# huangzh13/StyleGAN.pytorch

Hardware: AMD Instinct MI355X
Metric: img/s full G+D train step, 1024x1024 depth-9 bf16 (higher is better)
Workload: dtype bf16; 1 GPU; ffhq1024: StyleGAN 1024x1024, progressive depth index 8, logistic+R1, alpha 0.5, batch 4/GPU, global batch 4; global_batch=4, parallelism=dp1

## Files before the change

stylegan/pytorch_amd/csrc/pointwise.hip:

```cpp
#include "common.h"

static inline unsigned grid_for(size_t nvec, int block = 256) {
    size_t g = (nvec + block - 1) / block;
    static const size_t cap = [] { const char* e = getenv("SGX_GRID_CAP"); const long v = e ? atol(e) : 8192; return (size_t)(v > 0 ? v : 0x7fffffffL); }();
    if (g > cap) g = cap;
    if (g < 1) g = 1;
    return (unsigned)g;
}
static inline unsigned grid_all(size_t nvec, int block = 256) {
    size_t g = (nvec + block - 1) / block;
    static const size_t cap = [] { const char* e = getenv("SGX_GRID_ALL_CAP"); const long v = e ? atol(e) : 0; return (size_t)(v > 0 ? v : 0x7fffffffL); }();
    if (g > cap) g = cap;
    if (g < 1) g = 1;
    return (unsigned)g;
}

template <typename T>
__global__ void bias_act_kernel(const T* __restrict__ x, const float* __restrict__ bias, float bscale, T* __restrict__ y,
                                size_t nvec, int C, int act) {
    constexpr int VE = VecTraits<T>::VE;
    const int cv = C / VE;
    for (size_t i = (size_t)blockIdx.x * blockDim.x + threadIdx.x; i < nvec; i += (size_t)gridDim.x * blockDim.x) {
        float v[VE];
        VecTraits<T>::load(x + i * VE, v);
        const int c0 = (int)(i % cv) * VE;
#pragma unroll
        for (int j = 0; j < VE; ++j) {
            float t = v[j] + (bias ? bscale * bias[c0 + j] : 0.f);
            v[j] = act_apply(t, act);
        }
        VecTraits<T>::store(y + i * VE, v);
    }
}
__global__ void bias_act_scalar_kernel(const float* __restrict__ x, const float* __restrict__ bias, float bscale, float* __restrict__ y,
                                       size_t n, int C, int act) {
    for (size_t i = (size_t)blockIdx.x * blockDim.x + threadIdx.x; i < n; i += (size_t)gridDim.x * blockDim.x) {
        const float t = x[i] + (bias ? bscale * bias[i % C] : 0.f);
        y[i] = act_apply(t, act);
    }
}
extern "C" int sgx_bias_act(const void* x, const float* bias, float bscale, void* y, size_t npix, int C, int act, int dtype, void* stream) {
    hipStream_t st = (hipStream_t)stream;
    SGX_REQUIRE(act >= SGX_ACT_NONE && act <= SGX_ACT_RELU, SGX_EINVAL, "bias_act: activation %d", act);
    SGX_NOTE(0.0, 2.0 * (dtype == SGX_F32 ? 4.0 : 2.0) * npix * C, "bias_act %zux%d", npix, C);
    if (dtype == SGX_F32 && C % 4 != 0) {
        hipLaunchKernelGGL(bias_act_scalar_kernel, dim3(grid_for(npix * C)), dim3(256), 0, st, (const float*)x, bias, bscale, (float*)y, npix * C, C, act);
        SGX_LAUNCH_CHECK("bias_act_scalar");
        return 0;
    }
    if (dtype == SGX_F32) {
        SGX_REQUIRE(C % 4 == 0, SGX_EUNSUPPORTED, "bias_act: C %% 4");
        size_t nvec = npix * C / 4;
        hipLaunchKernelGGL(bias_act_kernel<float>, dim3(grid_all(nvec)), dim3(256), 0, st, (const float*)x, bias, bscale, (float*)y, nvec, C, act);
    } else {
// ... 11 lines not shown
    if (scale_dev) scale = scale_dev[0];
    constexpr int VE = VecTraits<T>::VE;
    for (size_t i = (size_t)blockIdx.x * blockDim.x + threadIdx.x; i < nvec; i += (size_t)gridDim.x * blockDim.x) {
        float g[VE], a[VE];
        VecTraits<T>::load(dy + i * VE, g);
        VecTraits<T>::load(y + i * VE, a);
#pragma unroll
        for (int j = 0; j < VE; ++j) g[j] = (scale * g[j]) * (a[j] > 0.f ? 1.f : slope);
        VecTraits<T>::store(dx + i * VE, g);
    }
}
extern "C" int sgx_lrelu_bwd(const void* dy, const void* y, void* dx, size_t n, float slope, float scale, const float* scale_dev, int dtype,
                             void* stream) {
    hipStream_t st = (hipStream_t)stream;
    SGX_NOTE(0.0, 3.0 * (dtype == SGX_F32 ? 4.0 : 2.0) * n, "lrelu_bwd %zu", n);
    if (dtype == SGX_F32) {
        SGX_REQUIRE(n % 4 == 0, SGX_EUNSUPPORTED, "lrelu_bwd: n %% 4");
        hipLaunchKernelGGL(lrelu_bwd_kernel<float>, dim3(grid_all(n / 4)), dim3(256), 0, st, (const float*)dy, (const float*)y, (float*)dx, n / 4, slope, scale, scale_dev);
    } else {
        SGX_REQUIRE(n % 8 == 0, SGX_EUNSUPPORTED, "lrelu_bwd: n %% 8");
        hipLaunchKernelGGL(lrelu_bwd_kernel<bf16_t>, dim3(grid_all(n / 8)), dim3(256), 0, st, (const bf16_t*)dy, (const bf16_t*)y, (bf16_t*)dx, n / 8, slope, scale, scale_dev);
    }
    SGX_LAUNCH_CHECK("lrelu_bwd");
    return 0;
}

__global__ void lrelu_bwd_bits_kernel(const bf16_t* __restrict__ dy, const unsigned char* __restrict__ bits, bf16_t* __restrict__ dx, size_t nvec, float slope,
                                      float scale, const float* __restrict__ scale_dev, int nt) {
    if (scale_dev) scale = scale_dev[0];
    for (size_t i = (size_t)blockIdx.x * blockDim.x + threadIdx.x; i < nvec; i += (size_t)gridDim.x * blockDim.x) {
        float g[8];
        const uint4 raw = ld16(dy + i * 8, nt != 0);
        const unsigned w4[4] = {raw.x, raw.y, raw.z, raw.w};
#pragma unroll
        for (int k = 0; k < 4; ++k) { g[2 * k] = __uint_as_float(w4[k] << 16); g[2 * k + 1] = __uint_as_float(w4[k] & 0xffff0000u); }
        const unsigned bb = bits[i];
#pragma unroll
        for (int j = 0; j < 8; ++j) g[j] = (scale * g[j]) * (((bb >> j) & 1u) ? 1.f : slope);
        st16(dx + i * 8, make_uint4(pack_bf16x2(g[0], g[1]), pack_bf16x2(g[2], g[3]), pack_bf16x2(g[4], g[5]), pack_bf16x2(g[6], g[7])), nt != 0);
    }
}
extern "C" int sgx_lrelu_bwd_bits(const void* dy, const void* bits, void* dx, size_t n, float slope, float scale, const float* scale_dev, int dtype,
                                  void* stream) {
    SGX_REQUIRE(dtype == SGX_BF16 && n % 8 == 0, SGX_EUNSUPPORTED, "lrelu_bwd_bits: bf16, n %% 8 == 0");
    SGX_REQUIRE(dy && bits && dx, SGX_EINVAL, "lrelu_bwd_bits: null argument");
    SGX_NOTE(0.0, 4.125 * n, "lrelu_bwd_bits %zu", n);
    hipLaunchKernelGGL(lrelu_bwd_bits_kernel, dim3(grid_all(n / 8)), dim3(256), 0, (hipStream_t)stream, (const bf16_t*)dy, (const unsigned char*)bits, (bf16_t*)dx,
                       n / 8, slope, scale, scale_dev, sgx_nt_for(2.0 * (double)n) ? 1 : 0);
    SGX_LAUNCH_CHECK("lrelu_bwd_bits");
    return 0;
}

#define FRB_BLOCKS 2048
template <int CV>
__global__ __launch_bounds__(256) void fade_rgb_bwd_kernel(const bf16_t* __restrict__ g, const unsigned char* __restrict__ bits, const float* __restrict__ pimg,
                                                           const float* __restrict__ wr, float ws, float alpha, float beta, const float* __restrict__ ab_dev,
                                                           bf16_t* __restrict__ gy, float* __restrict__ gpimg, double* __restrict__ part, size_t npix, int nt) {
    constexpr int PPI = 256 / CV;
    __shared__ double sh[4][CV][32];
    if (ab_dev) { alpha = ab_dev[0]; beta = ab_dev[1]; }
    const int tid = threadIdx.x, v = tid % CV, pl = tid / CV, lane = tid & 63, wave = tid >> 6;
    const size_t per = (npix + gridDim.x - 1) / gridDim.x;
    const size_t p0 = (size_t)blockIdx.x * per, p1 = p0 + per < npix ? p0 + per : npix;
    float wv[8][3];
    if (gpimg) {
#pragma unroll
        for (int j = 0; j < 8; ++j)
#pragma unroll
            for (int k = 0; k < 3; ++k) wv[j][k] = (beta * ws) * wr[(v * 8 + j) * 3 + k];
    }
    double acc[8][4];
    float q[8][4];
#pragma unroll
    for (int j = 0; j < 8; ++j)
#pragma unroll
        for (int k = 0; k < 4; ++k) { acc[j][k] = 0.0; q[j][k] = 0.f; }
    int cnt = 0;
    for (size_t pb = p0; pb < p1; pb += PPI) {
        const size_t p = pb + pl;
        const bool ok = p < p1;
        float gv[8];
        float i0 = 0.f, i1 = 0.f, i2 = 0.f;
        unsigned bb = 0;
        if (ok) {
            {
                const uint4 raw = ld16(g + (p * CV + v) * 8, nt != 0);
                const unsigned w4[4] = {raw.x, raw.y, raw.z, raw.w};
#pragma unroll
                for (int i = 0; i < 4; ++i) { gv[2 * i] = __uint_as_float(w4[i] << 16); gv[2 * i + 1] = __uint_as_float(w4[i] & 0xffff0000u); }
            }
            bb = bits[p * CV + v];
            i0 = pimg[p * 3]; i1 = pimg[p * 3 + 1]; i2 = pimg[p * 3 + 2];
            float o[8];
#pragma unroll
            for (int j = 0; j < 8; ++j) o[j] = (alpha * gv[j]) * (((bb >> j) & 1u) ? 1.f : SGX_LRELU);
            st16(gy + (p * CV + v) * 8, make_uint4(pack_bf16x2(o[0], o[1]), pack_bf16x2(o[2], o[3]), pack_bf16x2(o[4], o[5]), pack_bf16x2(o[6], o[7])), nt != 0);
        } else {
#pragma unroll
            for (int j = 0; j < 8; ++j) gv[j] = 0.f;
        }
#pragma unroll
        for (int j = 0; j < 8; ++j) { q[j][0] += gv[j] * i0; q[j][1] += gv[j] * i1; q[j][2] += gv[j] * i2; q[j][3] += gv[j]; }
        if (++cnt == 64) {
#pragma unroll
            for (int j = 0; j < 8; ++j)
#pragma unroll
                for (int k = 0; k < 4; ++k) { acc[j][k] += (double)q[j][k]; q[j][k] = 0.f; }
            cnt = 0;
        }
        if (gpimg) {
            float s0 = 0.f, s1 = 0.f, s2 = 0.f;
#pragma unroll
            for (int j = 0; j < 8; ++j) { s0 += gv[j] * wv[j][0]; s1 += gv[j] * wv[j][1]; s2 += gv[j] * wv[j][2]; }
#pragma unroll
            for (int o = 1; o < CV; o <<= 1) { s0 += __shfl_xor(s0, o, 64); s1 += __shfl_xor(s1, o, 64); s2 += __shfl_xor(s2, o, 64); }
            if (ok && v == 0) { gpimg[p * 3] = s0; gpimg[p * 3 + 1] = s1; gpimg[p * 3 + 2] = s2; }
        }
    }
#pragma unroll
    for (int j = 0; j < 8; ++j)
#pragma unroll
        for (int k = 0; k < 4; ++k) {
            double t = acc[j][k] + (double)q[j][k];
#pragma unroll
            for (int o = CV; o < 64; o <<= 1) t += __shfl_xor(t, o, 64);
            if (lane < CV) sh[wave][lane][j * 4 + k] = t;
        }
    __syncthreads();
    for (int e = tid; e < CV * 32; e += 256) {
        const int vv = e / 32, r = e % 32;
        part[((size_t)blockIdx.x * CV + vv) * 32 + r] = (sh[0][vv][r] + sh[1][vv][r]) + (sh[2][vv][r] + sh[3][vv][r]);
    }
}
__global__ __launch_bounds__(256) void fade_rgb_bwd_finish(const double* __restrict__ part, float* __restrict__ dw, float* __restrict__ drb, int nblk, int C,
                                                           float ws, float bs, float beta, const float* __restrict__ ab_dev, int acc) {
    __shared__ double sh[64][5];
    if (ab_dev) beta = ab_dev[1];
    const int el = threadIdx.x & 3, pl = threadIdx.x >> 2;
    const int e = blockIdx.x * 4 + el;
    double s = 0.0;
    if (e < 4 * C)
        for (int b = pl; b < nblk; b += 64) s += part[(size_t)b * 4 * C + e];
    sh[pl][el] = s;
    __syncthreads();
    if (pl == 0 && e < 4 * C) {
        double t = 0.0;
        for (int k = 0; k < 64; ++k) t += sh[k][el];
        const int c = e >> 2, j = e & 3;
        if (j < 3) {
            if (dw) { const float val = (float)(t * ((double)beta * (double)ws)); dw[c * 3 + j] = (acc & 1) ? dw[c * 3 + j] + val : val; }
        } else if (drb) {
            const float val = (float)(t * ((double)beta * (double)bs));
            drb[c] = (acc & 2) ? drb[c] + val : val;
        }
    }
}
extern "C" size_t sgx_fade_rgb_bwd_ws_bytes(size_t npix, int C) { (void)npix; return (size_t)FRB_BLOCKS * 4 * C * sizeof(double); }
extern "C" int sgx_fade_rgb_bwd(const void* g, const void* bits, const float* pimg, const float* wr, float ws, float bs, float alpha, float beta,
                                const float* ab_dev, void* gy, float* dwr, float* drb, int acc, float* gpimg, void* wsbuf, size_t ws_bytes, size_t npix, int C,
                                int dtype, void* stream) {
    SGX_REQUIRE(dtype == SGX_BF16 && (C == 32 || C == 64 || C == 128), SGX_EUNSUPPORTED, "fade_rgb_bwd: bf16, C in {32, 64, 128} (C=%d dtype %d)", C, dtype);
    SGX_REQUIRE(g && bits && pimg && wr && gy && wsbuf && npix > 0, SGX_EINVAL, "fade_rgb_bwd: null argument");
    SGX_REQUIRE(ws_bytes >= sgx_fade_rgb_bwd_ws_bytes(npix, C), SGX_EWORKSPACE, "fade_rgb_bwd: workspace");
    SGX_NOTE(8.0 * npix * C, npix * (4.125 * C + 12.0 + (gpimg ? 12.0 : 0.0)), "fade_rgb_bwd %zux%d", npix, C);
    hipStream_t st = (hipStream_t)stream;
    const int ppi = 256 / (C / 8);
    long nblk = (long)((npix + (size_t)ppi * 8 - 1) / ((size_t)ppi * 8));
    if (nblk > FRB_BLOCKS) nblk = FRB_BLOCKS;
    if (nblk < 1) nblk = 1;
    const bf16_t* gp = static_cast<const bf16_t*>(g);
    const unsigned char* bp = static_cast<const unsigned char*>(bits);
    bf16_t* yp = static_cast<bf16_t*>(gy);
    double* part = static_cast<double*>(wsbuf);
    const int nt = sgx_nt_for(2.0 * (double)npix * C) ? 1 : 0;
    if (C == 32) hipLaunchKernelGGL(fade_rgb_bwd_kernel<4>, dim3((unsigned)nblk), dim3(256), 0, st, gp, bp, pimg, wr, ws, alpha, beta, ab_dev, yp, gpimg, part, npix, nt);
    else if (C == 64) hipLaunchKernelGGL(fade_rgb_bwd_kernel<8>, dim3((unsigned)nblk), dim3(256), 0, st, gp, bp, pimg, wr, ws, alpha, beta, ab_dev, yp, gpimg, part, npix, nt);
    else hipLaunchKernelGGL(fade_rgb_bwd_kernel<16>, dim3((unsigned)nblk), dim3(256), 0, st, gp, bp, pimg, wr, ws, alpha, beta, ab_dev, yp, gpimg, part, npix, nt);
    SGX_LAUNCH_CHECK("fade_rgb_bwd_kernel");
    if (dwr || drb) {
        hipLaunchKernelGGL(fade_rgb_bwd_finish, dim3((unsigned)((4 * C + 3) / 4)), dim3(256), 0, st, part, dwr, drb, (int)nblk, C, ws, bs, beta, ab_dev, acc);
        SGX_LAUNCH_CHECK("fade_rgb_bwd_finish");
    }
    return 0;
}
extern "C" int sgx_fade_rgb_bwd_finish(const void* wsbuf, size_t ws_bytes, size_t npix, int C, float ws, float bs, float beta, const float* ab_dev,
                                       float* dwr, float* drb, int acc, void* stream) {
    SGX_REQUIRE(C == 32 || C == 64 || C == 128, SGX_EUNSUPPORTED, "fade_rgb_bwd_finish: C in {32, 64, 128} (C=%d)", C);
    SGX_REQUIRE(wsbuf && npix > 0 && (dwr || drb), SGX_EINVAL, "fade_rgb_bwd_finish: null argument");
    SGX_REQUIRE(ws_bytes >= sgx_fade_rgb_bwd_ws_bytes(npix, C), SGX_EWORKSPACE, "fade_rgb_bwd_finish: workspace");
    const int ppi = 256 / (C / 8);
    long nblk = (long)((npix + (size_t)ppi * 8 - 1) / ((size_t)ppi * 8));
    if (nblk > FRB_BLOCKS) nblk = FRB_BLOCKS;
    if (nblk < 1) nblk = 1;
    SGX_NOTE(0.0, (double)nblk * 4 * C * sizeof(double), "fade_rgb_bwd_finish C%d", C);
    hipLaunchKernelGGL(fade_rgb_bwd_finish, dim3((unsigned)((4 * C + 3) / 4)), dim3(256), 0, (hipStream_t)stream, static_cast<const double*>(wsbuf), dwr, drb,
                       (int)nblk, C, ws, bs, beta, ab_dev, acc);
    SGX_LAUNCH_CHECK("fade_rgb_bwd_finish");
    return 0;
}

__global__ __launch_bounds__(256) void fade_rgb_bwd2_kernel(const bf16_t* __restrict__ ggy, const float* __restrict__ ggp, const unsigned char* __restrict__ bits,
                                                            const float* __restrict__ wr, float ws, float alpha, float beta, const float* __restrict__ ab_dev,
                                                            bf16_t* __restrict__ out, size_t npix, int C) {
    const int cv = C / 8;
    const size_t nvec = npix * cv;
    const size_t i0 = (size_t)blockIdx.x * blockDim.x + threadIdx.x;
    const int c0 = (int)(i0 % cv) * 8;
    if (ab_dev) { alpha = ab_dev[0]; beta = ab_dev[1]; }
    float w0[8], w1[8], w2[8];
#pragma unroll
    for (int j = 0; j < 8; ++j) { w0[j] = ws * wr[(c0 + j) * 3]; w1[j] = ws * wr[(c0 + j) * 3 + 1]; w2[j] = ws * wr[(c0 + j) * 3 + 2]; }
    for (size_t i = i0; i < nvec; i += (size_t)gridDim.x * blockDim.x) {
        const size_t p = i / cv;
        float t1[8], t2[8], o[8];
#pragma unroll
        for (int j = 0; j < 8; ++j) { t1[j] = 0.f; t2[j] = 0.f; }
        if (ggy) {
            float g[8];
            VecTraits<bf16_t>::load(ggy + i * 8, g);
            const unsigned bb = bits[i];
#pragma unroll
            for (int j = 0; j < 8; ++j) t1[j] = bf2f(f2bf((alpha * g[j]) * (((bb >> j) & 1u) ? 1.f : SGX_LRELU)));
        }
        if (ggp) {
            const float r = ggp[p * 3], g = ggp[p * 3 + 1], b = ggp[p * 3 + 2];
#pragma unroll
            for (int j = 0; j < 8; ++j) {
                t2[j] = bf2f(f2bf(0.f + (r * w0[j] + g * w1[j] + b * w2[j])));
                if (ab_dev) t2[j] = bf2f(f2bf(beta * t2[j]));
            }
        }
#pragma unroll
        for (int j = 0; j < 8; ++j) o[j] = t1[j] + t2[j];
        VecTraits<bf16_t>::store(out + i * 8, o);
    }
}
extern "C" int sgx_fade_rgb_bwd2(const void* ggy, const float* ggp, const void* bits, const float* wr, float ws, float alpha, float beta, const float* ab_dev,
                                 void* out, size_t npix, int C, int dtype, void* stream) {
    SGX_REQUIRE(dtype == SGX_BF16 && (C == 32 || C == 64 || C == 128), SGX_EUNSUPPORTED, "fade_rgb_bwd2: bf16, C in {32, 64, 128} (C=%d dtype %d)", C, dtype);
    SGX_REQUIRE((ggy || ggp) && wr && out && npix > 0 && (!ggy || bits), SGX_EINVAL, "fade_rgb_bwd2: null argument");
    SGX_REQUIRE(ab_dev || beta == 1.0f, SGX_EUNSUPPORTED, "fade_rgb_bwd2: a host beta other than 1 rides in ws (as the forward's)");
    SGX_NOTE(6.0 * npix * C, npix * ((ggy ? 4.125 : 2.0) * C + (ggp ? 12.0 : 0.0)), "fade_rgb_bwd2 %zux%d", npix, C);
    const int cv = C / 8;
    unsigned grid = grid_for(npix * cv);
    hipLaunchKernelGGL(fade_rgb_bwd2_kernel, dim3(grid), dim3(256), 0, (hipStream_t)stream, static_cast<const bf16_t*>(ggy), ggp,
                       static_cast<const unsigned char*>(bits), wr, ws, alpha, beta, ab_dev, static_cast<bf16_t*>(out), npix, C);
    SGX_LAUNCH_CHECK("fade_rgb_bwd2_kernel");
    return 0;
}

template <typename T>
__global__ void axpby_kernel(const T* __restrict__ a, const T* __restrict__ b, T* __restrict__ out, float alpha, float beta,
                             const float* __restrict__ alpha_dev, const float* __restrict__ beta_dev, size_t nvec, size_t n) {
    constexpr int VE = VecTraits<T>::VE;
    if (alpha_dev) alpha = alpha_dev[0];
    if (beta_dev) beta = beta_dev[0];
    for (size_t i = (size_t)blockIdx.x * blockDim.x + threadIdx.x; i < nvec; i += (size_t)gridDim.x * blockDim.x) {
        if ((i + 1) * VE <= n) {
            float va[VE], vb[VE];
            VecTraits<T>::load(a + i * VE, va);
            if (b) {
                VecTraits<T>::load(b + i * VE, vb);
#pragma unroll
                for (int j = 0; j < VE; ++j) va[j] = alpha * va[j] + beta * vb[j];
            } else {
#pragma unroll
                for (int j = 0; j < VE; ++j) va[j] = alpha * va[j];
            }
            VecTraits<T>::store(out + i * VE, va);
        } else {
            for (size_t k = i * VE; k < n; ++k) {
                float t = alpha * to_f(a[k]) + (b ? beta * to_f(b[k]) : 0.f);
                out[k] = from_f<T>(t);
            }
        }
    }
}
static int axpby_launch(const void* a, const void* b, void* out, float alpha, float beta, const float* alpha_dev, const float* beta_dev,
                        size_t n, int dtype, void* stream) {
    hipStream_t st = (hipStream_t)stream;
    SGX_NOTE(0.0, (b ? 3.0 : 2.0) * (dtype == SGX_F32 ? 4.0 : 2.0) * n, "axpby %zu", n);
    if (n == 0) return 0;
    if (dtype == SGX_F32) {
        size_t nvec = (n + 3) / 4;
        hipLaunchKernelGGL(axpby_kernel<float>, dim3(grid_all(nvec)), dim3(256), 0, st, (const float*)a, (const float*)b, (float*)out, alpha, beta, alpha_dev, beta_dev, nvec, n);
    } else {
        size_t nvec = (n + 7) / 8;
        hipLaunchKernelGGL(axpby_kernel<bf16_t>, dim3(grid_all(nvec)), dim3(256), 0, st, (const bf16_t*)a, (const bf16_t*)b, (bf16_t*)out, alpha, beta, alpha_dev, beta_dev, nvec, n);
// ... 1041 lines not shown
    if (dtype == SGX_F32) hipLaunchKernelGGL(rgb_out_kernel<float>, dim3(g), dim3(256), sh, st, (const float*)x, w, sj, sc, wscale, bias, img, npix, C, lpp, low, H, W, alpha, beta, ab_dev);
    else hipLaunchKernelGGL(rgb_out_kernel<bf16_t>, dim3(g), dim3(256), sh, st, (const bf16_t*)x, w, sj, sc, wscale, bias, img, npix, C, lpp, low, H, W, alpha, beta, ab_dev);
    SGX_LAUNCH_CHECK("rgb_out");
    return 0;
}
extern "C" int sgx_rgb_out(const void* x, const float* w, int sj, int sc, float wscale, const float* bias, float* img, size_t npix, int C, int dtype, void* stream) {
    SGX_NOTE(6.0 * npix * C, npix * (12.0 + (dtype == SGX_F32 ? 4.0 : 2.0) * C), "rgb_out %zux%d", npix, C);
    return rgb_out_launch(x, w, sj, sc, wscale, bias, img, npix, C, dtype, nullptr, 1, 1, 1.f, 0.f, nullptr, (hipStream_t)stream);
}
extern "C" int sgx_rgb_out_fade(const void* x, const float* w, int sj, int sc, float wscale, const float* bias, const float* low, float alpha,
                                float beta, const float* ab_dev, float* img, int B, int H, int W, int C, int dtype, void* stream) {
    SGX_REQUIRE(x && w && low && img && B > 0 && H > 0 && W > 0 && H % 2 == 0 && W % 2 == 0, SGX_EINVAL, "rgb_out_fade: bad arguments (%dx%d)", H, W);
    const size_t npix = (size_t)B * H * W;
    SGX_NOTE(6.0 * npix * C, npix * (12.0 + 3.0 + (dtype == SGX_F32 ? 4.0 : 2.0) * C), "rgb_out+fade %zux%d", npix, C);
    return rgb_out_launch(x, w, sj, sc, wscale, bias, img, npix, C, dtype, low, H, W, alpha, beta, ab_dev, (hipStream_t)stream);
}

template <typename T>
__global__ __launch_bounds__(256) void rgb_out_epi_kernel(const T* __restrict__ y, const float* __restrict__ ebias, const float* __restrict__ noise,
                                                          const float* __restrict__ nw, const float* __restrict__ style, const float* __restrict__ mean,
                                                          const float* __restrict__ rstd, const float* __restrict__ w, int sj, int sc, float wscale,
                                                          const float* __restrict__ rbias, float* __restrict__ img, int HW, int C, int lpp,
                                                          const float* __restrict__ low, int Himg, int Wimg, float alpha, float beta,
                                                          const float* __restrict__ ab_dev) {
    constexpr int VE = VecTraits<T>::VE;
    extern __shared__ float sw[];
    if (ab_dev) { alpha = ab_dev[0]; beta = ab_dev[1]; }
    float* kb = sw + 3 * C; float* kw = kb + C; float* sb = kw + C; float* red = sb + 4;
    const int b = blockIdx.y;
    float c0 = 0.f, c1 = 0.f, c2 = 0.f;
    for (int c = threadIdx.x; c < C; c += blockDim.x) {
        const float s0 = style ? style[(size_t)b * 2 * C + c] : 0.f, s1 = style ? style[(size_t)b * 2 * C + C + c] : 0.f;
        const float A = rstd[(size_t)b * C + c] * (s0 + 1.f), S = s1 - mean[(size_t)b * C + c] * A;
        const float w0 = (alpha * wscale) * w[c * sc], w1 = (alpha * wscale) * w[sj + c * sc], w2 = (alpha * wscale) * w[2 * sj + c * sc];
        sw[c] = w0 * A; sw[C + c] = w1 * A; sw[2 * C + c] = w2 * A;
        c0 += w0 * S; c1 += w1 * S; c2 += w2 * S;
        kb[c] = ebias ? ebias[c] : 0.f; kw[c] = nw[c];
    }
    red[threadIdx.x * 3] = c0; red[threadIdx.x * 3 + 1] = c1; red[threadIdx.x * 3 + 2] = c2;
    __syncthreads();
    if (threadIdx.x < 3) {
        float t = 0.f;
        for (int k = 0; k < 256; ++k) t += red[k * 3 + threadIdx.x];
        sb[threadIdx.x] = t + (rbias ? alpha * rbias[threadIdx.x] : 0.f);
    }
    __syncthreads();
    const float b0 = sb[0], b1 = sb[1], b2 = sb[2];
    const int cv = C / VE;
    const int sub = threadIdx.x % lpp;
    const int gid = (blockIdx.x * blockDim.x + threadIdx.x) / lpp, gstride = (gridDim.x * blockDim.x) / lpp;
    const T* yb = y + (size_t)b * HW * C;
    const float* nzb = noise + (size_t)b * HW;
    const int niter = (HW + gstride - 1) / gstride;
    for (int it = 0; it < niter; ++it) {
        const int p = gid + it * gstride;
        float s0 = 0.f, s1 = 0.f, s2 = 0.f;
        if (p < HW) {
            const float nz = nzb[p];
            for (int v = sub; v < cv; v += lpp) {
                float t[VE];
                VecTraits<T>::load(yb + ((size_t)p * cv + v) * VE, t);
#pragma unroll
                for (int q = 0; q < VE; ++q) {
                    const int c = v * VE + q;
                    const float a = lrelu(t[q] + kb[c] + kw[c] * nz);
                    s0 += a * sw[c]; s1 += a * sw[C + c]; s2 += a * sw[2 * C + c];
                }
            }
        }
        for (int o = lpp >> 1; o > 0; o >>= 1) {
            s0 += __shfl_xor(s0, o, 64); s1 += __shfl_xor(s1, o, 64); s2 += __shfl_xor(s2, o, 64);
        }
        if (p < HW && sub == 0) {
            float o0 = s0 + b0, o1 = s1 + b1, o2 = s2 + b2;
            if (low) {
                const int xw = p % Wimg, yy = p / Wimg;
                const float* l = low + (((size_t)b * (Himg >> 1) + (yy >> 1)) * (Wimg >> 1) + (xw >> 1)) * 3;
                o0 += beta * l[0]; o1 += beta * l[1]; o2 += beta * l[2];
            }
            float* o = img + ((size_t)b * HW + p) * 3;
            o[0] = o0; o[1] = o1; o[2] = o2;
        }
    }
}
extern "C" int sgx_rgb_out_epi(const void* y, const float* ebias, const float* noise, const float* nw, const float* style, const float* mean,
                               const float* rstd, const float* w, int sj, int sc, float wscale, const float* rbias, const float* low, float alpha,
                               float beta, const float* ab_dev, float* img, int B, int H, int W, int C, int dtype, void* stream) {
    SGX_REQUIRE(y && noise && nw && mean && rstd && w && img && B > 0 && H > 0 && W > 0, SGX_EINVAL, "rgb_out_epi: bad arguments");
    SGX_REQUIRE(!low || (H % 2 == 0 && W % 2 == 0), SGX_EINVAL, "rgb_out_epi: odd size %dx%d with a low-resolution image", H, W);
    const int ve = dtype == SGX_F32 ? 4 : 8;
    SGX_REQUIRE((dtype == SGX_F32 || dtype == SGX_BF16) && C % ve == 0 && C <= 2048, SGX_EUNSUPPORTED, "rgb_out_epi: C=%d", C);
    int lpp = C / ve;
    if (lpp > 16) lpp = 16;
    SGX_REQUIRE((lpp & (lpp - 1)) == 0, SGX_EUNSUPPORTED, "rgb_out_epi: C=%d", C);
    const int HW = H * W;
    const double npix = (double)B * HW;
    SGX_NOTE(8.0 * npix * C, npix * (12.0 + 4.0 + (low ? 3.0 : 0.0) + (dtype == SGX_F32 ? 4.0 : 2.0) * C), "epi+rgb_out%s %.0fx%d", low ? "+fade" : "", npix, C);
    long bx = ((long)HW * lpp + 255) / 256;
    const long cap = 4096 / B > 1 ? 4096 / B : 1;
    if (bx > cap) bx = cap;
    const size_t sh = (size_t)(5 * C + 4 + 256 * 3) * sizeof(float);
    hipStream_t st = (hipStream_t)stream;
    if (dtype == SGX_F32)
        hipLaunchKernelGGL(rgb_out_epi_kernel<float>, dim3((unsigned)bx, (unsigned)B), dim3(256), sh, st, (const float*)y, ebias, noise, nw, style, mean, rstd, w, sj, sc,
                           wscale, rbias, img, HW, C, lpp, low, H, W, alpha, beta, ab_dev);
    else
// ... 179 lines not shown
```

stylegan/pytorch_amd/csrc/rgbconv.hip:

```cpp
#include "common.h"
#include <stdlib.h>

typedef __attribute__((ext_vector_type(4))) float f32x4_t;

typedef _Float16 h16x4 __attribute__((ext_vector_type(4)));
typedef _Float16 h16x2 __attribute__((ext_vector_type(2)));
typedef float f32x2 __attribute__((ext_vector_type(2)));
static __device__ __forceinline__ unsigned pack_f16x2(float lo, float hi) {
    const h16x2 v = {(_Float16)lo, (_Float16)hi};
    return __builtin_bit_cast(unsigned, v);
}
static __device__ __forceinline__ f32x4_t mma16h(s16x4 a, s16x4 b, f32x4_t c) {
    return __builtin_amdgcn_mfma_f32_16x16x16f16(__builtin_bit_cast(h16x4, a), __builtin_bit_cast(h16x4, b), c, 0, 0, 0);
}
static __device__ __forceinline__ f32x4_t mma16(s16x4 a, s16x4 b, f32x4_t c) {
    return __builtin_amdgcn_mfma_f32_16x16x16bf16_1k(a, b, c, 0, 0, 0);
}

__global__ void rgbconv_pack_kernel(const float* __restrict__ w0, float s0, const float* __restrict__ wr, float sr,
                                    const float* __restrict__ br, float bscale, bf16_t* __restrict__ wf, bf16_t* __restrict__ wd, int C) {
    const int tid = threadIdx.x + blockIdx.x * blockDim.x, nth = blockDim.x * gridDim.x;
    for (int e = tid; e < 3 * C * 16; e += nth) {
        const int ky = e / (C * 16), o = (e / 16) % C, k = e % 16, kx = k >> 2, j = k & 3;
        float v = 0.f;
// ... 294 lines not shown
                    a[2 * q] = fmaxf(p.x, n.x); a[2 * q + 1] = fmaxf(p.y, n.y);
                }
                unsigned nib = 0u;
#pragma unroll
                for (int i = 0; i < 4; ++i)
                    nib |= (unsigned)min(max(__float_as_int(a[i]), 0), 1) << i;
                const auto sw = __builtin_amdgcn_permlane16_swap(nib, nib, false, false);
                float h[4];
#pragma unroll
                for (int i = 0; i < 4; ++i) {
                    const float t = a[i] + dpp_row_shr1(a[i]);
                    h[i] = t + dpp_row_shl1(t);
                }
                const f32x2 vc0 = f32x2{h1[cb][0], h1[cb][1]} + f32x2{h[0], h[1]}, vc1 = f32x2{h1[cb][2], h1[cb][3]} + f32x2{h[2], h[3]};
                if (store_row) {
                    if (y_out) {
                        const f32x2 o0 = vp[cb][0] + vc0, o1 = vp[cb][1] + vc1;
                        *reinterpret_cast<uint2*>(yrow + yoff + cb * 16) = make_uint2(pack_bf16x2(o0.x, o0.y), pack_bf16x2(o1.x, o1.y));
                    }
                    if (bit_out) brow[boff + cb * 2] = (unsigned char)pbyte[cb];
                }
                vp[cb][0] = vc0; vp[cb][1] = vc1;
#pragma unroll
                for (int i = 0; i < 4; ++i) h1[cb][i] = h[i];
                pbyte[cb] = sw[0] | (sw[1] << 4);
            }
        }
    }
}
template <int CB>
__global__ __launch_bounds__(256) void rgbconv_fwdblur_kernel(const float* __restrict__ img, const bf16_t* __restrict__ wf, const float* __restrict__ b0,
                                                              bf16_t* __restrict__ y, unsigned char* __restrict__ bits, int B, int H, int W, int ones,
                                                              int nstrips, int nrb, int nit, int dbg) {
    constexpr int C = 16 * CB;
    int item = __builtin_amdgcn_readfirstlane((int)(rc_xcd_block() * 4 + (threadIdx.x >> 6)));
    const int sx = item % nstrips; item /= nstrips;
    const int rbk = item % nrb, b = item / nrb;
    if (b >= B) return;
    const int rb = 6 * nit - 2;
    const int r_begin = rbk * rb, r_end = r_begin + rb < H ? r_begin + rb : H;
    const float* ibase = img + (size_t)b * H * W * 3;
    bf16_t* ybase = y + (size_t)b * H * W * C;
    unsigned char* bbase = bits ? bits + (size_t)b * H * W * (C / 8) : nullptr;
    const bool inside = sx * RC_STRIP - 2 >= 0 && sx * RC_STRIP + 15 < W && r_begin - 2 >= 0 && r_begin + rb + 1 < H;
    if (inside) fwdblur_walk<CB, false>(ibase, wf, b0, ybase, bbase, H, W, ones, sx, r_begin, r_end, nit, dbg);
    else fwdblur_walk<CB, true>(ibase, wf, b0, ybase, bbase, H, W, ones, sx, r_begin, r_end, nit, dbg);
}

template <int CB>
__global__ __launch_bounds__(256) void rgbconv_dgrad_kernel(const bf16_t* __restrict__ gz, const bf16_t* __restrict__ wd, float* __restrict__ gi,
                                                            int B, int H, int W, int nstrips, int nrb) {
    constexpr int C = 16 * CB;
    const int lane = threadIdx.x & 63, l15 = lane & 15, l4 = lane >> 4;
    int item = (int)rc_xcd_block() * 4 + (threadIdx.x >> 6);
    const int sx = item % nstrips; item /= nstrips;
    const int rbk = item % nrb, b = item / nrb;
    if (b >= B) return;
    const int r_begin = rbk * RC_ROWS, r_end = r_begin + RC_ROWS < H ? r_begin + RC_ROWS : H;
    const int pc = sx * RC_STRIP - 1 + l15;
    const bool pc_ok = (unsigned)pc < (unsigned)W;
    s16x4 wfr[3][CB];
#pragma unroll
    for (int ky = 0; ky < 3; ++ky)
#pragma unroll
        for (int cb = 0; cb < CB; ++cb) wfr[ky][cb] = *reinterpret_cast<const s16x4*>(wd + ((ky * 16 + l15) * C + cb * 16 + 4 * l4));
    const bf16_t* gbase = gz + (size_t)b * H * W * C;
    struct Row { uint2 v[CB]; };
    auto load_row = [&](int gy) -> Row {
        Row r;
#pragma unroll
        for (int cb = 0; cb < CB; ++cb) {
            r.v[cb] = make_uint2(0u, 0u);
            if (pc_ok && (unsigned)gy < (unsigned)H) r.v[cb] = *reinterpret_cast<const uint2*>(gbase + ((size_t)gy * W + pc) * C + cb * 16 + 4 * l4);
        }
        return r;
    };
    auto frag_of = [&](const uint2& u) -> s16x4 {
        s16x4 f;
        f[0] = (short)(u.x & 0xffffu); f[1] = (short)(u.x >> 16); f[2] = (short)(u.y & 0xffffu); f[3] = (short)(u.y >> 16);
        return f;
    };
    Row g0 = load_row(r_begin - 1), g1 = load_row(r_begin);
    Row ring[RC_PF];
#pragma unroll
    for (int u = 0; u < RC_PF; ++u) ring[u] = load_row(r_begin + 1 + u);
    const bool col_out = l4 == 1 && l15 >= 1 && l15 <= RC_STRIP && pc < W;
    for (int rb = r_begin; rb < r_end; rb += RC_PF) {
#pragma unroll
        for (int u = 0; u < RC_PF; ++u) {
            const int r = rb + u;
            if (r < r_end) {
                const Row g2 = ring[u];
                ring[u] = load_row(r + 1 + RC_PF);
                f32x4_t acc = f32x4_t{0.f, 0.f, 0.f, 0.f};
#pragma unroll
                for (int cb = 0; cb < CB; ++cb) {
                    acc = mma16(wfr[0][cb], frag_of(g0.v[cb]), acc);
                    acc = mma16(wfr[1][cb], frag_of(g1.v[cb]), acc);
                    acc = mma16(wfr[2][cb], frag_of(g2.v[cb]), acc);
                }
                float o3[3];
#pragma unroll
                for (int j = 0; j < 3; ++j) o3[j] = __shfl(acc[j], l15 - 1, 64) + acc[j] + __shfl(acc[j], 32 + l15 + 1, 64);
                if (col_out) *reinterpret_cast<rgb3*>(gi + (((size_t)b * H + r) * W + pc) * 3) = rgb3{o3[0], o3[1], o3[2]};
                g0 = g1; g1 = g2;
            }
        }
    }
}

template <int CB> struct RcWg {
    static constexpr int C = 16 * CB, TH = 8, TW = 64, TP = TH * TW, RH = TH + 2;
    static constexpr int TPS = TP + 8, IPS = RH * TW + 8;
    static constexpr int GZT = C * TPS * 2;
    static constexpr int IMT = 12 * IPS * 2;
    static constexpr int RED = 4 * CB * 3 * 256 * 4;
    static constexpr int LDS = (GZT + IMT > RED ? GZT + IMT : RED);
    static constexpr int NOUT = C * 48;
};

template <int CB>
__global__ __launch_bounds__(256) void rgbconv_wgrad_kernel(const float* __restrict__ img, const bf16_t* __restrict__ gz, float* __restrict__ part,
                                                            int B, int H, int W, int ones, int tiles_x, int tiles_y, int ntiles) {
    using G = RcWg<CB>;
    constexpr int C = G::C, TH = G::TH, TW = G::TW, TP = G::TP, TPS = G::TPS, IPS = G::IPS, RH = G::RH, VPP = C / 8;
    extern __shared__ __attribute__((aligned(16))) char smem[];
    bf16_t* gzT = reinterpret_cast<bf16_t*>(smem);
    bf16_t* imgT = reinterpret_cast<bf16_t*>(smem + G::GZT);
    const int tid = threadIdx.x, lane = tid & 63, wave = tid >> 6, l15 = lane & 15, l4 = lane >> 4;
    f32x4_t acc[CB][3];
#pragma unroll
    for (int cb = 0; cb < CB; ++cb)
#pragma unroll
        for (int ky = 0; ky < 3; ++ky) acc[cb][ky] = f32x4_t{0.f, 0.f, 0.f, 0.f};
    const int nkx = (l15 >> 2) < 3 ? (l15 >> 2) : 0, nj = l15 & 3;
    const RcSched sc = rc_sched(ntiles);
    constexpr int NGV = TP * VPP / 256;
    constexpr int NIP = RH * (TW + 2), NII = (NIP + 255) / 256;
    uint4 gv[NGV];
    rgb3 iv[NII];
    unsigned okm = 0;
    auto tile_at = [&](int t, int& b, int& ty0, int& tx0) {
        const int tx = t % tiles_x; t /= tiles_x;
        const int ty = t % tiles_y;
        b = t / tiles_y; ty0 = ty * TH; tx0 = tx * TW;
    };
    auto load_tile = [&](int t) {
        int b, ty0, tx0;
        tile_at(t, b, ty0, tx0);
#pragma unroll
        for (int it = 0; it < NGV; ++it) {
            const int idx = it * 256 + tid, p = idx / VPP, v = idx - p * VPP, r = p / TW, c = p - r * TW;
            const int gy = ty0 + r, gx = tx0 + c;
            gv[it] = (gy < H && gx < W) ? *reinterpret_cast<const uint4*>(gz + (((size_t)b * H + gy) * W + gx) * C + v * 8) : make_uint4(0u, 0u, 0u, 0u);
        }
        okm = 0;
#pragma unroll
        for (int it = 0; it < NII; ++it) {
            const int idx = it * 256 + tid, rr = idx / (TW + 2), cr = idx - rr * (TW + 2);
// ... 268 lines not shown
```

Measured before the change: 283.1 img/s.

## Unroll and batch loads in fade-RGB, to-RGB and rgbconv dgrad kernels

Several RGB-path kernels get restructured for more memory-level parallelism. fade_rgb_bwd and fade_rgb_bwd2 now issue loads for several pixel trips before computing, with compile-time variants for full tiles and for the nt and nullable-input cases. fade_rgb_bwd also moves its weights into shared memory and uses DPP lane swizzles for the small reductions. A to-RGB kernel gains an unrolled fast path when the channel split matches, and rgbconv dgrad clamps its addresses so loads are branch-free, masking the out-of-range values afterwards. These changes add more registers and code, and the unconditional dgrad loop runs extra MMA work on tail rows.

```diff
diff --git a/stylegan/pytorch_amd/csrc/pointwise.hip b/stylegan/pytorch_amd/csrc/pointwise.hip
--- a/stylegan/pytorch_amd/csrc/pointwise.hip
+++ b/stylegan/pytorch_amd/csrc/pointwise.hip
@@ -1,5 +1,12 @@
 #include "common.h"
-
+#include <type_traits>
+
+template <int O>
+__device__ __forceinline__ float lane_xor(float v) {
+    if constexpr (O == 1) return __int_as_float(__builtin_amdgcn_mov_dpp(__float_as_int(v), 0xB1, 0xf, 0xf, true));
+    else if constexpr (O == 2) return __int_as_float(__builtin_amdgcn_mov_dpp(__float_as_int(v), 0x4E, 0xf, 0xf, true));
+    else return __shfl_xor(v, O, 64);
+}
 static inline unsigned grid_for(size_t nvec, int block = 256) {
     size_t g = (nvec + block - 1) / block;
     static const size_t cap = [] { const char* e = getenv("SGX_GRID_CAP"); const long v = e ? atol(e) : 8192; return (size_t)(v > 0 ? v : 0x7fffffffL); }();
@@ -117,84 +124,137 @@
 }
 
 #define FRB_BLOCKS 2048
+#define FRB_U 2
+#define FRB_US 4
 template <int CV>
 __global__ __launch_bounds__(256) void fade_rgb_bwd_kernel(const bf16_t* __restrict__ g, const unsigned char* __restrict__ bits, const float* __restrict__ pimg,
                                                            const float* __restrict__ wr, float ws, float alpha, float beta, const float* __restrict__ ab_dev,
                                                            bf16_t* __restrict__ gy, float* __restrict__ gpimg, double* __restrict__ part, size_t npix, int nt) {
     constexpr int PPI = 256 / CV;
     __shared__ double sh[4][CV][32];
+    __shared__ float wv[CV][24];
     if (ab_dev) { alpha = ab_dev[0]; beta = ab_dev[1]; }
     const int tid = threadIdx.x, v = tid % CV, pl = tid / CV, lane = tid & 63, wave = tid >> 6;
     const size_t per = (npix + gridDim.x - 1) / gridDim.x;
     const size_t p0 = (size_t)blockIdx.x * per, p1 = p0 + per < npix ? p0 + per : npix;
-    float wv[8][3];
     if (gpimg) {
+        for (int e = tid; e < CV * 24; e += 256) wv[e / 24][e % 24] = (beta * ws) * wr[e];
+        __syncthreads();
+    }
+    float q[8][4];
+#pragma unroll
+    for (int j = 0; j < 8; ++j)
+#pragma unroll
+        for (int k = 0; k < 4; ++k) q[j][k] = 0.f;
+    auto trips = [&](auto UC, auto NT, auto FULL, size_t pb, auto&& flush) {
+        constexpr int UU = decltype(UC)::value;
+        constexpr bool nth = decltype(NT)::value;
+        constexpr bool full = decltype(FULL)::value;
+        uint4 raw[UU];
+        unsigned bb[UU];
+        float im[UU][3];
+        const uint4* gb = reinterpret_cast<const uint4*>(g) + pb * CV;
+        const unsigned char* bq = bits + pb * CV;
+        const float* ib = pimg + pb * 3;
+#pragma unroll
+        for (int u = 0; u < UU; ++u) {
+            const unsigned pi = (unsigned)(u * PPI + pl);
+            const bool ok = full || pb + pi < p1;
+            const unsigned pc = ok ? pi : (unsigned)(p1 - 1 - pb);
+            const uint4 r = ld16(gb + (pc * CV + v), nth);
+            bb[u] = bq[pc * CV + v];
+            const float a0 = ib[pc * 3], a1 = ib[pc * 3 + 1], a2 = ib[pc * 3 + 2];
+            raw[u] = make_uint4(ok ? r.x : 0u, ok ? r.y : 0u, ok ? r.z : 0u, ok ? r.w : 0u);
+            im[u][0] = ok ? a0 : 0.f; im[u][1] = ok ? a1 : 0.f; im[u][2] = ok ? a2 : 0.f;
+        }
+#pragma unroll
+        for (int u = 0; u < UU; ++u) {
+            const unsigned pi = (unsigned)(u * PPI + pl);
+            const bool ok = full || pb + pi < p1;
+            float gv[8];
+            const unsigned w4[4] = {raw[u].x, raw[u].y, raw[u].z, raw[u].w};
+#pragma unroll
+            for (int i = 0; i < 4; ++i) { gv[2 * i] = __uint_as_float(w4[i] << 16); gv[2 * i + 1] = __uint_as_float(w4[i] & 0xffff0000u); }
+            const float i0 = im[u][0], i1 = im[u][1], i2 = im[u][2];
+            if (ok) {
+                float o[8];
+#pragma unroll
+                for (int j = 0; j < 8; ++j) o[j] = (alpha * gv[j]) * (((bb[u] >> j) & 1u) ? 1.f : SGX_LRELU);
+                st16(reinterpret_cast<uint4*>(gy) + pb * CV + (pi * CV + v),
+                     make_uint4(pack_bf16x2(o[0], o[1]), pack_bf16x2(o[2], o[3]), pack_bf16x2(o[4], o[5]), pack_bf16x2(o[6], o[7])), nth);
+            }
+#pragma unroll
+            for (int j = 0; j < 8; ++j) { q[j][0] += gv[j] * i0; q[j][1] += gv[j] * i1; q[j][2] += gv[j] * i2; q[j][3] += gv[j]; }
+            flush();
+            if (gpimg) {
+                float s0 = 0.f, s1 = 0.f, s2 = 0.f;
+#pragma unroll
+                for (int j = 0; j < 8; ++j) { s0 += gv[j] * wv[v][j * 3]; s1 += gv[j] * wv[v][j * 3 + 1]; s2 += gv[j] * wv[v][j * 3 + 2]; }
+                if constexpr (CV > 1) { s0 += lane_xor<1>(s0); s1 += lane_xor<1>(s1); s2 += lane_xor<1>(s2); }
+                if constexpr (CV > 2) { s0 += lane_xor<2>(s0); s1 += lane_xor<2>(s1); s2 += lane_xor<2>(s2); }
+                if constexpr (CV > 4) { s0 += lane_xor<4>(s0); s1 += lane_xor<4>(s1); s2 += lane_xor<4>(s2); }
+                if constexpr (CV > 8) { s0 += lane_xor<8>(s0); s1 += lane_xor<8>(s1); s2 += lane_xor<8>(s2); }
+                if (ok && v == 0) { float* o = gpimg + pb * 3 + pi * 3; o[0] = s0; o[1] = s1; o[2] = s2; }
+            }
+        }
+    };
+    const size_t span = p0 < p1 ? p1 - p0 : 0, ntrip = (span + PPI - 1) / PPI, nfull = span / PPI;
+    auto walk = [&](auto UC, auto NT, auto&& flush) {
+        constexpr int UU = decltype(UC)::value;
+        size_t t = 0;
+        for (; t + UU <= nfull; t += UU) trips(UC, NT, std::true_type{}, p0 + t * PPI, flush);
+        if constexpr (UU > 2)
+            for (; t + 2 <= nfull; t += 2) trips(std::integral_constant<int, 2>{}, NT, std::true_type{}, p0 + t * PPI, flush);
+        for (; t < ntrip; ++t) trips(std::integral_constant<int, 1>{}, NT, std::false_type{}, p0 + t * PPI, flush);
+    };
+    auto finish = [&](auto&& total) {
+        double t[8][4];
 #pragma unroll
         for (int j = 0; j < 8; ++j)
 #pragma unroll
-            for (int k = 0; k < 3; ++k) wv[j][k] = (beta * ws) * wr[(v * 8 + j) * 3 + k];
-    }
-    double acc[8][4];
-    float q[8][4];
-#pragma unroll
-    for (int j = 0; j < 8; ++j)
-#pragma unroll
-        for (int k = 0; k < 4; ++k) { acc[j][k] = 0.0; q[j][k] = 0.f; }
-    int cnt = 0;
-    for (size_t pb = p0; pb < p1; pb += PPI) {
-        const size_t p = pb + pl;
-        const bool ok = p < p1;
-        float gv[8];
-        float i0 = 0.f, i1 = 0.f, i2 = 0.f;
-        unsigned bb = 0;
-        if (ok) {
-            {
-                const uint4 raw = ld16(g + (p * CV + v) * 8, nt != 0);
-                const unsigned w4[4] = {raw.x, raw.y, raw.z, raw.w};
-#pragma unroll
-                for (int i = 0; i < 4; ++i) { gv[2 * i] = __uint_as_float(w4[i] << 16); gv[2 * i + 1] = __uint_as_float(w4[i] & 0xffff0000u); }
-            }
-            bb = bits[p * CV + v];
-            i0 = pimg[p * 3]; i1 = pimg[p * 3 + 1]; i2 = pimg[p * 3 + 2];
-            float o[8];
-#pragma unroll
-            for (int j = 0; j < 8; ++j) o[j] = (alpha * gv[j]) * (((bb >> j) & 1u) ? 1.f : SGX_LRELU);
-            st16(gy + (p * CV + v) * 8, make_uint4(pack_bf16x2(o[0], o[1]), pack_bf16x2(o[2], o[3]), pack_bf16x2(o[4], o[5]), pack_bf16x2(o[6], o[7])), nt != 0);
-        } else {
-#pragma unroll
-            for (int j = 0; j < 8; ++j) gv[j] = 0.f;
-        }
-#pragma unroll
-        for (int j = 0; j < 8; ++j) { q[j][0] += gv[j] * i0; q[j][1] += gv[j] * i1; q[j][2] += gv[j] * i2; q[j][3] += gv[j]; }
-        if (++cnt == 64) {
+            for (int k = 0; k < 4; ++k) t[j][k] = total(j, k);
+#pragma unroll
+        for (int o = CV; o < 64; o <<= 1)
 #pragma unroll
             for (int j = 0; j < 8; ++j)
 #pragma unroll
-                for (int k = 0; k < 4; ++k) { acc[j][k] += (double)q[j][k]; q[j][k] = 0.f; }
-            cnt = 0;
-        }
-        if (gpimg) {
-            float s0 = 0.f, s1 = 0.f, s2 = 0.f;
-#pragma unroll
-            for (int j = 0; j < 8; ++j) { s0 += gv[j] * wv[j][0]; s1 += gv[j] * wv[j][1]; s2 += gv[j] * wv[j][2]; }
-#pragma unroll
-            for (int o = 1; o < CV; o <<= 1) { s0 += __shfl_xor(s0, o, 64); s1 += __shfl_xor(s1, o, 64); s2 += __shfl_xor(s2, o, 64); }
-            if (ok && v == 0) { gpimg[p * 3] = s0; gpimg[p * 3 + 1] = s1; gpimg[p * 3 + 2] = s2; }
-        }
-    }
-#pragma unroll
-    for (int j = 0; j < 8; ++j)
-#pragma unroll
-        for (int k = 0; k < 4; ++k) {
-            double t = acc[j][k] + (double)q[j][k];
-#pragma unroll
-            for (int o = CV; o < 64; o <<= 1) t += __shfl_xor(t, o, 64);
-            if (lane < CV) sh[wave][lane][j * 4 + k] = t;
-        }
-    __syncthreads();
-    for (int e = tid; e < CV * 32; e += 256) {
-        const int vv = e / 32, r = e % 32;
-        part[((size_t)blockIdx.x * CV + vv) * 32 + r] = (sh[0][vv][r] + sh[1][vv][r]) + (sh[2][vv][r] + sh[3][vv][r]);
+                for (int k = 0; k < 4; ++k) t[j][k] += __shfl_xor(t[j][k], o, 64);
+        if (lane < CV) {
+#pragma unroll
+            for (int j = 0; j < 8; ++j)
+#pragma unroll
+                for (int k = 0; k < 4; ++k) sh[wave][lane][j * 4 + k] = t[j][k];
+        }
+        __syncthreads();
+        for (int e = tid; e < CV * 32; e += 256) {
+            const int vv = e / 32, r = e % 32;
+            part[((size_t)blockIdx.x * CV + vv) * 32 + r] = (sh[0][vv][r] + sh[1][vv][r]) + (sh[2][vv][r] + sh[3][vv][r]);
+        }
+    };
+    if (ntrip < 64) {
+        auto none = [] {};
+        if (nt) walk(std::integral_constant<int, FRB_US>{}, std::true_type{}, none);
+        else walk(std::integral_constant<int, FRB_US>{}, std::false_type{}, none);
+        finish([&](int j, int k) { return 0.0 + (double)q[j][k]; });
+    } else {
+        double acc[8][4];
+#pragma unroll
+        for (int j = 0; j < 8; ++j)
+#pragma unroll
+            for (int k = 0; k < 4; ++k) acc[j][k] = 0.0;
+        int cnt = 0;
+        auto flush = [&] {
+            if (++cnt == 64) {
+#pragma unroll
+                for (int j = 0; j < 8; ++j)
+#pragma unroll
+                    for (int k = 0; k < 4; ++k) { acc[j][k] += (double)q[j][k]; q[j][k] = 0.f; }
+                cnt = 0;
+            }
+        };
+        if (nt) walk(std::integral_constant<int, FRB_U>{}, std::true_type{}, flush);
+        else walk(std::integral_constant<int, FRB_U>{}, std::false_type{}, flush);
+        finish([&](int j, int k) { return acc[j][k] + (double)q[j][k]; });
     }
 }
 __global__ __launch_bounds__(256) void fade_rgb_bwd_finish(const double* __restrict__ part, float* __restrict__ dw, float* __restrict__ drb, int nblk, int C,
@@ -275,30 +335,54 @@
     float w0[8], w1[8], w2[8];
 #pragma unroll
     for (int j = 0; j < 8; ++j) { w0[j] = ws * wr[(c0 + j) * 3]; w1[j] = ws * wr[(c0 + j) * 3 + 1]; w2[j] = ws * wr[(c0 + j) * 3 + 2]; }
-    for (size_t i = i0; i < nvec; i += (size_t)gridDim.x * blockDim.x) {
-        const size_t p = i / cv;
-        float t1[8], t2[8], o[8];
-#pragma unroll
-        for (int j = 0; j < 8; ++j) { t1[j] = 0.f; t2[j] = 0.f; }
-        if (ggy) {
-            float g[8];
-            VecTraits<bf16_t>::load(ggy + i * 8, g);
-            const unsigned bb = bits[i];
-#pragma unroll
-            for (int j = 0; j < 8; ++j) t1[j] = bf2f(f2bf((alpha * g[j]) * (((bb >> j) & 1u) ? 1.f : SGX_LRELU)));
-        }
-        if (ggp) {
-            const float r = ggp[p * 3], g = ggp[p * 3 + 1], b = ggp[p * 3 + 2];
-#pragma unroll
-            for (int j = 0; j < 8; ++j) {
-                t2[j] = bf2f(f2bf(0.f + (r * w0[j] + g * w1[j] + b * w2[j])));
-                if (ab_dev) t2[j] = bf2f(f2bf(beta * t2[j]));
-            }
-        }
-#pragma unroll
-        for (int j = 0; j < 8; ++j) o[j] = t1[j] + t2[j];
-        VecTraits<bf16_t>::store(out + i * 8, o);
-    }
+    const size_t gs = (size_t)gridDim.x * blockDim.x;
+    const int cvs = __ffs(cv) - 1;
+    auto trips = [&](auto UC, auto HY, auto HP, size_t i) {
+        constexpr int UU = decltype(UC)::value;
+        constexpr bool hy = decltype(HY)::value, hp = decltype(HP)::value;
+        uint4 raw[UU];
+        unsigned bb[UU];
+        float pr[UU], pg[UU], pb[UU];
+#pragma unroll
+        for (int u = 0; u < UU; ++u) {
+            const size_t iu = i + u * gs;
+            if constexpr (hy) { raw[u] = *reinterpret_cast<const uint4*>(ggy + iu * 8); bb[u] = bits[iu]; }
+            if constexpr (hp) { const size_t p = iu >> cvs; pr[u] = ggp[p * 3]; pg[u] = ggp[p * 3 + 1]; pb[u] = ggp[p * 3 + 2]; }
+        }
+#pragma unroll
+        for (int u = 0; u < UU; ++u) {
+            float t1[8], t2[8], o[8];
+#pragma unroll
+            for (int j = 0; j < 8; ++j) { t1[j] = 0.f; t2[j] = 0.f; }
+            if constexpr (hy) {
+                const unsigned w4[4] = {raw[u].x, raw[u].y, raw[u].z, raw[u].w};
+                float g[8];
+#pragma unroll
+                for (int k = 0; k < 4; ++k) { g[2 * k] = __uint_as_float(w4[k] << 16); g[2 * k + 1] = __uint_as_float(w4[k] & 0xffff0000u); }
+#pragma unroll
+                for (int j = 0; j < 8; ++j) t1[j] = bf2f(f2bf((alpha * g[j]) * (((bb[u] >> j) & 1u) ? 1.f : SGX_LRELU)));
+            }
+            if constexpr (hp) {
+                const float r = pr[u], g = pg[u], b = pb[u];
+#pragma unroll
+                for (int j = 0; j < 8; ++j) {
+                    t2[j] = bf2f(f2bf(0.f + (r * w0[j] + g * w1[j] + b * w2[j])));
+                    if (ab_dev) t2[j] = bf2f(f2bf(beta * t2[j]));
+                }
+            }
+#pragma unroll
+            for (int j = 0; j < 8; ++j) o[j] = t1[j] + t2[j];
+            VecTraits<bf16_t>::store(out + (i + u * gs) * 8, o);
+        }
+    };
+    auto walk = [&](auto HY, auto HP) {
+        size_t i = i0;
+        for (; i + gs < nvec; i += 2 * gs) trips(std::integral_constant<int, 2>{}, HY, HP, i);
+        if (i < nvec) trips(std::integral_constant<int, 1>{}, HY, HP, i);
+    };
+    if (ggy && ggp) walk(std::true_type{}, std::true_type{});
+    else if (ggy) walk(std::true_type{}, std::false_type{});
+    else walk(std::false_type{}, std::true_type{});
 }
 extern "C" int sgx_fade_rgb_bwd2(const void* ggy, const float* ggp, const void* bits, const float* wr, float ws, float alpha, float beta, const float* ab_dev,
                                  void* out, size_t npix, int C, int dtype, void* stream) {
@@ -1446,6 +1530,60 @@
     const T* yb = y + (size_t)b * HW * C;
     const float* nzb = noise + (size_t)b * HW;
     const int niter = (HW + gstride - 1) / gstride;
+    if (cv == lpp) {
+        float rb[VE], rw[VE], r0[VE], r1[VE], r2[VE];
+#pragma unroll
+        for (int q = 0; q < VE; ++q) { const int c = sub * VE + q; rb[q] = kb[c]; rw[q] = kw[c]; r0[q] = sw[c]; r1[q] = sw[C + c]; r2[q] = sw[2 * C + c]; }
+        auto trips = [&](auto UC, int it) {
+            constexpr int UU = decltype(UC)::value;
+            uint4 raw[UU];
+            float nz[UU], lo[UU][3];
+#pragma unroll
+            for (int u = 0; u < UU; ++u) {
+                const int p = gid + (it + u) * gstride;
+                const int pc = p < HW ? p : HW - 1;
+                nz[u] = nzb[pc];
+                raw[u] = *reinterpret_cast<const uint4*>(yb + ((size_t)pc * cv + sub) * VE);
+                if (low) {
+                    const int xw = pc % Wimg, yy = pc / Wimg;
+                    const float* l = low + (((size_t)b * (Himg >> 1) + (yy >> 1)) * (Wimg >> 1) + (xw >> 1)) * 3;
+                    lo[u][0] = l[0]; lo[u][1] = l[1]; lo[u][2] = l[2];
+                }
+            }
+#pragma unroll
+            for (int u = 0; u < UU; ++u) {
+                const int p = gid + (it + u) * gstride;
+                float t[VE];
+                const unsigned w4[4] = {raw[u].x, raw[u].y, raw[u].z, raw[u].w};
+                if constexpr (sizeof(T) == 2) {
+#pragma unroll
+                    for (int k = 0; k < 4; ++k) { t[(2 * k) % VE] = __uint_as_float(w4[k] << 16); t[(2 * k + 1) % VE] = __uint_as_float(w4[k] & 0xffff0000u); }
+                } else {
+#pragma unroll
+                    for (int k = 0; k < 4; ++k) t[k % VE] = __uint_as_float(w4[k]);
+                }
+                float s0 = 0.f, s1 = 0.f, s2 = 0.f;
+#pragma unroll
+                for (int q = 0; q < VE; ++q) {
+                    const float a = lrelu(t[q] + rb[q] + rw[q] * nz[u]);
+                    s0 += a * r0[q]; s1 += a * r1[q]; s2 += a * r2[q];
+                }
+                for (int o = lpp >> 1; o > 0; o >>= 1) {
+                    s0 += __shfl_xor(s0, o, 64); s1 += __shfl_xor(s1, o, 64); s2 += __shfl_xor(s2, o, 64);
+                }
+                if (p < HW && sub == 0) {
+                    float o0 = s0 + b0, o1 = s1 + b1, o2 = s2 + b2;
+                    if (low) { o0 += beta * lo[u][0]; o1 += beta * lo[u][1]; o2 += beta * lo[u][2]; }
+                    float* o = img + ((size_t)b * HW + p) * 3;
+                    o[0] = o0; o[1] = o1; o[2] = o2;
+                }
+            }
+        };
+        int it = 0;
+        for (; it + 2 <= niter; it += 2) trips(std::integral_constant<int, 2>{}, it);
+        if (it < niter) trips(std::integral_constant<int, 1>{}, it);
+        return;
+    }
     for (int it = 0; it < niter; ++it) {
         const int p = gid + it * gstride;
         float s0 = 0.f, s1 = 0.f, s2 = 0.f;
diff --git a/stylegan/pytorch_amd/csrc/rgbconv.hip b/stylegan/pytorch_amd/csrc/rgbconv.hip
--- a/stylegan/pytorch_amd/csrc/rgbconv.hip
+++ b/stylegan/pytorch_amd/csrc/rgbconv.hip
@@ -370,7 +370,7 @@
                                                             int B, int H, int W, int nstrips, int nrb) {
     constexpr int C = 16 * CB;
     const int lane = threadIdx.x & 63, l15 = lane & 15, l4 = lane >> 4;
-    int item = (int)rc_xcd_block() * 4 + (threadIdx.x >> 6);
+    int item = __builtin_amdgcn_readfirstlane((int)rc_xcd_block() * 4 + (int)(threadIdx.x >> 6));
     const int sx = item % nstrips; item /= nstrips;
     const int rbk = item % nrb, b = item / nrb;
     if (b >= B) return;
@@ -384,14 +384,20 @@
         for (int cb = 0; cb < CB; ++cb) wfr[ky][cb] = *reinterpret_cast<const s16x4*>(wd + ((ky * 16 + l15) * C + cb * 16 + 4 * l4));
     const bf16_t* gbase = gz + (size_t)b * H * W * C;
     struct Row { uint2 v[CB]; };
+    const int pcc = pc < 0 ? 0 : (pc < W ? pc : W - 1);
     auto load_row = [&](int gy) -> Row {
         Row r;
-#pragma unroll
-        for (int cb = 0; cb < CB; ++cb) {
-            r.v[cb] = make_uint2(0u, 0u);
-            if (pc_ok && (unsigned)gy < (unsigned)H) r.v[cb] = *reinterpret_cast<const uint2*>(gbase + ((size_t)gy * W + pc) * C + cb * 16 + 4 * l4);
-        }
+        const int gyc = gy < 0 ? 0 : (gy < H ? gy : H - 1);
+#pragma unroll
+        for (int cb = 0; cb < CB; ++cb) r.v[cb] = *reinterpret_cast<const uint2*>(gbase + ((size_t)gyc * W + pcc) * C + cb * 16 + 4 * l4);
         return r;
+    };
+    auto zero_outside = [&](const Row& r, int gy) -> Row {
+        const bool ok = pc_ok && (unsigned)gy < (unsigned)H;
+        Row z;
+#pragma unroll
+        for (int cb = 0; cb < CB; ++cb) z.v[cb] = make_uint2(ok ? r.v[cb].x : 0u, ok ? r.v[cb].y : 0u);
+        return z;
     };
     auto frag_of = [&](const uint2& u) -> s16x4 {
         s16x4 f;
@@ -402,27 +408,26 @@
     Row ring[RC_PF];
 #pragma unroll
     for (int u = 0; u < RC_PF; ++u) ring[u] = load_row(r_begin + 1 + u);
+    g0 = zero_outside(g0, r_begin - 1); g1 = zero_outside(g1, r_begin);
     const bool col_out = l4 == 1 && l15 >= 1 && l15 <= RC_STRIP && pc < W;
     for (int rb = r_begin; rb < r_end; rb += RC_PF) {
 #pragma unroll
         for (int u = 0; u < RC_PF; ++u) {
             const int r = rb + u;
-            if (r < r_end) {
-                const Row g2 = ring[u];
-                ring[u] = load_row(r + 1 + RC_PF);
-                f32x4_t acc = f32x4_t{0.f, 0.f, 0.f, 0.f};
-#pragma unroll
-                for (int cb = 0; cb < CB; ++cb) {
-                    acc = mma16(wfr[0][cb], frag_of(g0.v[cb]), acc);
-                    acc = mma16(wfr[1][cb], frag_of(g1.v[cb]), acc);
-                    acc = mma16(wfr[2][cb], frag_of(g2.v[cb]), acc);
-                }
-                float o3[3];
-#pragma unroll
-                for (int j = 0; j < 3; ++j) o3[j] = __shfl(acc[j], l15 - 1, 64) + acc[j] + __shfl(acc[j], 32 + l15 + 1, 64);
-                if (col_out) *reinterpret_cast<rgb3*>(gi + (((size_t)b * H + r) * W + pc) * 3) = rgb3{o3[0], o3[1], o3[2]};
-                g0 = g1; g1 = g2;
-            }
+            const Row g2 = zero_outside(ring[u], r + 1);
+            ring[u] = load_row(r + 1 + RC_PF);
+            f32x4_t acc = f32x4_t{0.f, 0.f, 0.f, 0.f};
+#pragma unroll
+            for (int cb = 0; cb < CB; ++cb) {
+                acc = mma16(wfr[0][cb], frag_of(g0.v[cb]), acc);
+                acc = mma16(wfr[1][cb], frag_of(g1.v[cb]), acc);
+                acc = mma16(wfr[2][cb], frag_of(g2.v[cb]), acc);
+            }
+            float o3[3];
+#pragma unroll
+            for (int j = 0; j < 3; ++j) o3[j] = __shfl(acc[j], l15 - 1, 64) + acc[j] + __shfl(acc[j], 32 + l15 + 1, 64);
+            if (col_out && r < r_end) *reinterpret_cast<rgb3*>(gi + (((size_t)b * H + r) * W + pc) * 3) = rgb3{o3[0], o3[1], o3[2]};
+            g0 = g1; g1 = g2;
         }
     }
 }
```

Result: no change. 285.1 img/s, median of 6 (+0.7%).
